# drapado/PINGS

Measured on AMD Instinct MI355X. Metric: raster fwd+bwd Mpix/s @1M Gaussians 1080p, higher is better.
Workload: dtype f32; 1 GPU; surfel rasteriser fwd+bwd, 1000000 Gaussians, 1920x1080, one view per GPU; gaussians=1000000, width=1920, height=1080

## Files before the change

include/pings_hip.h:

```cpp
#ifndef PINGS_HIP_H_
#define PINGS_HIP_H_

#include <stddef.h>
#include <stdint.h>

#if defined(__cplusplus)
#define PINGS_EXTERN_C extern "C"
#else
#define PINGS_EXTERN_C
#endif
#define PINGS_API PINGS_EXTERN_C __attribute__((visibility("default")))

#define PINGS_OK 0
#define PINGS_ERR_ARG 1
#define PINGS_ERR_HIP 2
#define PINGS_ERR_CAPACITY 3


#define PINGS_ABI_VERSION 11
PINGS_API int pings_abi_version(void);
PINGS_API const char* pings_last_error(void);

PINGS_API int pings_prof_enable(int on);
PINGS_API int pings_prof_only(const char* stage);
// ... 79 lines not shown
                                    void* bwd_blob, float* dL_dmeans3D, float* dL_dmeans2D,
                                    float* dL_dcolors, float* dL_dopacities, float* dL_dscales,
                                    float* dL_drotations, float* dL_dtau, int footprint_class,
                                    void* stream);

PINGS_API int pings_raster_debug_lists(const void* binning_blob, int64_t num_instances,
                                       int image_height, int image_width, uint32_t* point_list,
                                       uint32_t* ranges_xy, void* stream);
PINGS_API int pings_raster_debug_image(const void* image_blob, int image_height, int image_width,
                                       float* final_T, uint32_t* n_contrib, void* stream);
PINGS_API int pings_raster_debug_occlusion(const void* geom_blob, int P, int image_height, int image_width,
                                           uint32_t* occ_bucket, uint16_t* occ_bsat, int32_t* occ_nb,
                                           void* stream);
PINGS_API int pings_raster_rank_bucket(const int32_t* ranks, int64_t n, int occ_nb, uint32_t nvalid,
                                       uint32_t* buckets);
PINGS_API int pings_raster_debug_interior(const float* records, const float* tile_origins, int64_t n, float cxp,
                                          float cyp, float fx, float fy, uint8_t* flags);


PINGS_API size_t pings_raster2d_geom_bytes(int P, int image_height, int image_width);
PINGS_API size_t pings_raster2d_binning_bytes(int64_t num_instances, int image_height, int image_width);
PINGS_API size_t pings_raster2d_image_bytes(int image_height, int image_width);

PINGS_API int pings_raster2d_preprocess(const pings_raster_settings* s, int P, const float* means3D,
                                        const float* colors, const float* opacities, const float* scales,
                                        const float* rotations, void* geom_blob, int32_t* radii,
                                        const int32_t* live_rows_dev, int dyn_rows, const int32_t* const* aux_dev,
                                        int aux_words, int32_t* aux_host, int64_t* num_instances, void* stream);

PINGS_API int pings_raster2d_render(const pings_raster_settings* s, int P, int64_t num_instances, void* geom_blob,
// ... 814 lines not shown
```

pings_amd/_abi.py:

```python
from __future__ import annotations

import ctypes as C

ABI_VERSION = 11

RASTER_SURFEL, RASTER_3DGS, RASTER_2DGS = 0, 1, 2
HEAD_COLOR, HEAD_SEMANTIC = 0, 1
REG_SINGULAR, REG_ILL_CONDITIONED, REG_NONFINITE = 1, 2, 4
REG_F_NORMALS, REG_F_DIV_GRAD, REG_F_WEIGHTED = 1, 2, 4
REG_COLOR_PHOTO, REG_COLOR_CONSIST = 1, 2
MC_ALLOW_DEGENERATE, MC_ASCENT = 1, 2
ADAMW_MAX_JOBS, ADAMW_CHUNK = 48, 4096
EVAL_VIEW_RECORD, EVAL_PAIR_RECORD = 9, 12
EVAL_EXTENT = 1
MESH_SAMPLE_UNIT_BITS, MESH_SAMPLE_SUM_BITS = 32, 62
MESH_SAMPLE_INDEX, MESH_SAMPLE_NONFINITE, MESH_SAMPLE_AREA_CAP = 16, 32, 64
LOOP_MAX_R, LOOP_MAX_S, LOOP_MAX_D = 32, 128, 16
LOOP_MAX_Q, LOOP_MAX_C = 16, 65536
LIDAR_MAX_CAMS, LIDAR_MAX_LIDARS = 8, 8
CAMFRONT_MAX_MAPS, CAMFRONT_TILE_W, CAMFRONT_TILE_H = 32, 128, 32
CAMFRONT_RGB_U8, CAMFRONT_RGB_F32, CAMFRONT_NORMAL, CAMFRONT_DEPTH, CAMFRONT_SKY = 0, 1, 2, 3, 4
CAMFRONT_FIT_RECORD, CAMFRONT_MIN_FIT = 5, 100
CAMFRONT_FULL = 2
TSDF_BLOCK = 8
# ... 186 lines not shown
                                      C.POINTER(i32), vp]),
    "pings_raster_preprocess_dyn": (i32, [C.POINTER(RasterSettings), i32, vp, vp, vp, vp, vp, vp, vp, vp, i32,
                                          C.POINTER(vp), i32, C.POINTER(i32), C.POINTER(i64), C.POINTER(i32), vp]),
    "pings_raster_render": (i32, [C.POINTER(RasterSettings), i32, i64, vp, vp, vp, vp, vp, vp, vp, vp, i32, vp]),
    "pings_raster_tile_sort_bytes": (sz, [i64, C.POINTER(i32)]),
    "pings_raster_tile_sort": (i32, [vp, i64, i32, i32, vp, vp, vp, i32, vp]),
    "pings_raster_scan_bytes": (sz, [i64]),
    "pings_raster_scan_u32": (i32, [vp, i64, i32, i32, vp, vp, sz, vp]),
    "pings_raster_backward_bytes": (sz, [i32, i64]),
    "pings_raster_backward": (i32, [C.POINTER(RasterSettings), i32, i64, vp, vp, vp, vp, vp, vp, vp, vp, vp, vp, vp, vp,
                                    vp, vp, vp, vp, vp, vp, vp, vp, vp, vp, vp, vp, i32, vp]),
    "pings_raster_debug_lists": (i32, [vp, i64, i32, i32, vp, vp, vp]),
    "pings_raster_debug_image": (i32, [vp, i32, i32, vp, vp, vp]),
    "pings_raster_debug_occlusion": (i32, [vp, i32, i32, i32, vp, vp, C.POINTER(C.c_int32), vp]),
    "pings_raster_rank_bucket": (i32, [vp, i64, i32, C.c_uint32, vp]),
    "pings_raster_debug_interior": (i32, [vp, vp, i64, f32, f32, f32, f32, vp]),
    "pings_raster2d_geom_bytes": (sz, [i32, i32, i32]),
    "pings_raster2d_binning_bytes": (sz, [i64, i32, i32]),
    "pings_raster2d_image_bytes": (sz, [i32, i32]),
    "pings_raster2d_preprocess": (i32, [C.POINTER(RasterSettings), i32, vp, vp, vp, vp, vp, vp, vp, vp, i32,
                                        C.POINTER(vp), i32, C.POINTER(i32), C.POINTER(i64), vp]),
    "pings_raster2d_render": (i32, [C.POINTER(RasterSettings), i32, i64, vp, vp, vp, vp, vp, vp]),
    "pings_raster2d_backward_bytes": (sz, [i32, i64]),
    "pings_raster2d_backward": (i32, [C.POINTER(RasterSettings), i32, i64, vp, vp, vp, vp, vp, vp, vp, vp, vp, vp, vp,
                                      vp, vp, vp, vp]),
    "pings_raster2d_debug_lists": (i32, [vp, i64, i32, i32, vp, vp, vp]),
    "pings_raster2d_debug_image": (i32, [vp, i32, i32, vp, vp, vp, vp]),
    "pings_knn_compact_entries": (sz, [i64]),
    "pings_knn_compact_build": (i32, [vp, i64, vp, sz, vp]),
    "pings_knn_blocks_entries": (sz, [i64]),
# ... 192 lines not shown
```

pings_amd/csrc/raster_common.hpp:

```cpp
#pragma once
#include <cmath>
#include <cstdlib>
#include <type_traits>

#include "common.hpp"

namespace pings {
namespace raster {

constexpr int TILE = 16;
constexpr int BLOCK = TILE * TILE;
constexpr float NEAR_Z = 0.2f;
constexpr float LOWPASS = 0.3f;
constexpr float ALPHA_MAX = 0.99f;
constexpr float ALPHA_MIN = 1.0f / 255.0f;
constexpr float T_EPS = 1e-4f;
constexpr float DEPTH_ALPHA_EPS = 1e-10f;
constexpr float DEN_EPS = 1e-6f;
constexpr uint32_t CULLED_KEY = 0xFFFFFFFFu;
constexpr int DS_NB = 1 << 20;
constexpr uint32_t DS_LIMIT = 4096u;
constexpr int DS_SHARDS = 64;
constexpr int DS_KMIN = 2 * DS_SHARDS, DS_SHIFT = DS_KMIN + 1, DS_FLAG = DS_KMIN + 2, DS_HEAD = DS_KMIN + 8;
constexpr int STAT_SHARDS = 256;
// ... 5 lines not shown
constexpr uint16_t OCC_ALL = 0xFFFFu;

constexpr int MODE_SURFEL = 0;
constexpr int MODE_3DGS = 1;
constexpr int RECT_TIGHT = 0, RECT_3SIGMA = 1, RECT_ELLIPSE = 2;

constexpr int GRAD_ROW = 16;
constexpr int CH = 64;
enum GradSlot {
  G_MX = 0, G_MY = 1, G_CONX = 2, G_CONY = 3, G_CONZ = 4, G_OPAC = 5,
  G_R = 6, G_G = 7, G_B = 8, G_NX = 9, G_NY = 10, G_NZ = 11, G_Q = 12, G_PZ = 13,
  G_ZLO = 14, G_ZHI = 15
};

struct FrameSummary {
  uint32_t overflow, pad0;
  unsigned long long stats[3];
  int32_t aux[8];
  uint32_t seq;
  uint32_t pad;
};

struct GeomState {
  float4* rec;
  uint4* rect;
  uint32_t *depth_key, *depth_key_sorted, *gidx, *gidx_sorted;
  uint32_t* rank_of;
  uint32_t *tiles_sorted, *offsets_sorted;
  uint32_t* occ_bucket;
  uint16_t* occ_bsat;
  unsigned long long* occ_mask;
  uint32_t* nvalid;
  uint32_t* occ_bmax;
  uint32_t* ds_head;
  uint32_t *ds_cnt, *ds_fill, *ds_off;
  char* zero_begin; size_t zero_bytes;
  size_t ds_words;
  uint32_t* ds_idx;
  unsigned long long* stats;
  FrameSummary* summary;
  int occ_nb, occ_words;
  char* temp;
  size_t temp_bytes;
  size_t total;
};

struct BinState {
  uint32_t *tile_key, *tile_key_sorted, *gval, *point_list;
// ... 86 lines not shown
  uint32_t blend_seg = 512u;
  bool seg_reuse = true;
  uint32_t bwd_long = 3072u;
  bool occlusion = true;
  bool library_sort = false;
  bool library_tile_sort = false;
  bool library_scan = false;
  float occ_amin = 0.15f;
  bool occ_walk_lanes = false;
  int rect_rule = RECT_TIGHT;
  bool mark_depth_only = false;
  unsigned rowsum_wgs = 2048u;
  unsigned grad_fill_wgs = 512u;
  bool chain_sum_lanes = false;
  bool blend_interior = true;
};
RasterKnobs read_knobs();

struct BlendPlan {
  enum Fwd { FWD_TILE, FWD_WAVE } fwd;
  bool want_qmask;
  bool bwd_scan;
  uint32_t seg;
  bool seg_on, seg_reuse;
  uint32_t long_thr;
  bool interior_bwd;
};
BlendPlan blend_plan(const RasterKnobs& k, int footprint_class, int64_t I, int num_tiles);

struct BwdState {
// ... 11 lines not shown
                      uint32_t long_thr = 0, uint32_t long_max = 0);
int occlusion_buckets(int num_tiles);
BinState carve_binning(void* blob, int64_t I, int num_tiles, uint32_t seg);
ImageState carve_image(void* blob, int W, int H);
BwdState carve_bwd(void* blob, int P, int64_t I);

constexpr int TS_THREADS = 256, TS_BLOCK = 4096;
size_t tile_sort_table_bytes(int64_t n);
template <typename KeyT>
int tile_sort(const KeyT* keys_in, int64_t n, int bits, KeyT* keys_tmp, uint32_t* vals_tmp, KeyT* keys_out,
              uint32_t* vals_out, uint32_t* table, hipStream_t st);
size_t tile_sort_library_bytes(int64_t n);
template <typename KeyT>
int tile_sort_library(const KeyT* keys_in, int64_t n, int bits, KeyT* keys_out, uint32_t* vals_out, void* temp,
                      size_t temp_bytes, hipStream_t st);

int launch_blend_fwd(int mode, const KParams& kp, const BlendPlan& plan, int P, int64_t I, const GeomState& gs,
                     const BinState& bs, const ImageState& im, float* out_color, float* out_normal, float* out_depth,
                     float* out_alpha, void* per_gaussian, hipStream_t st);

__device__ inline int lane_value(int v, int src) { return __builtin_amdgcn_readlane(v, src); }
__device__ inline uint32_t lane_value(uint32_t v, int src) { return (uint32_t)__builtin_amdgcn_readlane((int)v, src); }
__device__ inline float lane_value(float v, int src) {
  return __builtin_bit_cast(float, __builtin_amdgcn_readlane(__builtin_bit_cast(int, v), src));
}

__device__ inline int dealt_rank(int num_waves, int wave, int lane) {
  return lane < 16 ? lane * num_waves + wave : ((lane >> 4) * num_waves + wave) * 16 + (lane & 15);
}
__device__ inline int strided_rank(int P) {
// ... 13 lines not shown
  uint32_t J = 0u;
  if ((eq >> RB_LW) != 0u) {
    J = rank_bucket_log2(eq >> RB_LW) + 2u;
    if (J > (unb >> (RB_LS + 1))) J = unb >> (RB_LS + 1);
  }
  const uint32_t front_ranks = J ? 1u << (RB_LW + RB_LS + J - 1u) : 0u, front_buckets = J << RB_LS;
  if (ur < front_ranks) {
    const uint32_t q = ur >> RB_LW;
    if ((q >> RB_LS) == 0u) return q;
    const uint32_t k = rank_bucket_log2(q) - RB_LS;
    return (k << RB_LS) + (q >> k);
  }
  const uint32_t b = front_buckets + (uint32_t)(((unsigned long long)(ur - front_ranks) * (unb - front_buckets)) /
                                                (unsigned long long)(nvalid - front_ranks));
  return b < unb ? b : unb - 1u;
}

typedef float f2 __attribute__((ext_vector_type(2)));
__device__ inline f2 f2s(float x) { return f2{x, x}; }
__device__ inline f2 fma2(f2 a, f2 b, f2 c) { return __builtin_elementwise_fma(a, b, c); }
__device__ inline f2 mul_rounded(f2 a, f2 b) {
#pragma clang fp contract(off)
  return a * b;
}
__device__ inline f2 sel2(bool c0, bool c1, f2 a, f2 b) { return f2{c0 ? a.x : b.x, c1 ? a.y : b.y}; }

typedef unsigned long long lmask;
struct cmask {
  unsigned long long bits;
};
// ... 390 lines not shown
```

pings_amd/csrc/raster_fwd.hip:

```cpp
#include <hipcub/hipcub.hpp>

#include <algorithm>
#include <chrono>
#include <type_traits>

#include "raster_common.hpp"

namespace pings {
namespace raster {

__device__ inline void to_camera(const float* __restrict__ V, float x, float y, float z, float& px,
                                 float& py, float& pz) {
  px = ((V[0] * x + V[4] * y) + V[8] * z) + V[12];
  py = ((V[1] * x + V[5] * y) + V[9] * z) + V[13];
  pz = ((V[2] * x + V[6] * y) + V[10] * z) + V[14];
}

__global__ __launch_bounds__(256) void mark_visible_kernel(const float* __restrict__ pos, int N,
                                                            const float* __restrict__ V,
                                                            const float* __restrict__ Pm,
                                                            uint8_t* __restrict__ present, int depth_only) {
  const int i = blockIdx.x * blockDim.x + threadIdx.x;
  if (i >= N) return;
  float px, py, pz;
// ... 254 lines not shown
  if (r >= 0 && (uint32_t)r < nvalid) {
    me.g = gidx_sorted[r];
    const uint4 rc = rect[me.g];
    me.n = rc.w;
    me.xmin = (int)(rc.y & 0xFFFF);
    me.ymin = (int)(rc.y >> 16);
    me.wdt = max((int)(rc.z & 0xFFFF) - me.xmin, 1);
    me.hgt = max((int)(rc.z >> 16) - me.ymin, 1);
  }
  return me;
}

constexpr int SMALL_ITEMS = 16;
constexpr uint32_t SMALL_KEPT = 16u;

__device__ inline unsigned long long kept_bits(const unsigned long long* __restrict__ m, int s, int w) {
  const int i = s >> 6, sh = s & 63;
  const unsigned long long lo = m[i], hi = m[i + 1];
  const unsigned long long v = sh ? (lo >> sh) | (hi << (64 - sh)) : lo;
  return v & (~0ull >> (64 - w));
}

struct RowItems {
  int s0, gx, wdt, cpr;
  float inv_cpr;
  __device__ RowItems(int xmin, int ymin, int wdt_, int gx_)
      : s0(ymin * gx_ + xmin), gx(gx_), wdt(wdt_), cpr((wdt_ + 63) >> 6), inv_cpr(1.0f / (float)((wdt_ + 63) >> 6)) {}
  __device__ void at(uint32_t k, int& s, int& w) const {
    int y = (int)k, c = 0;
    if (cpr > 1) {
      y = (int)((float)k * inv_cpr);
      c = (int)k - y * cpr;
      if (c < 0) { --y; c += cpr; }
      if (c >= cpr) { ++y; c -= cpr; }
    }
    s = s0 + y * gx + 64 * c;
// ... 444 lines not shown
                     n_long, long_thr, long_max);
  PINGS_LAUNCH_CHECK();
  return PINGS_OK;
}

template <typename KeyT>
__global__ __launch_bounds__(256) void tile_ranges_kernel(int64_t I, const KeyT* __restrict__ key,
                                                           uint2* __restrict__ ranges) {
  const int64_t i = (int64_t)blockIdx.x * blockDim.x + threadIdx.x;
  if (i >= I) return;
  const uint32_t t = (uint32_t)key[i];
  if (i == 0 || key[i - 1] != t) ranges[t].x = (uint32_t)i;
  if (i == I - 1 || key[i + 1] != t) ranges[t].y = (uint32_t)(i + 1);
}

struct AuxPtrs {
  const int32_t* p[8];
};
__global__ __launch_bounds__(64) void frame_summary_kernel(const uint32_t* __restrict__ overflow,
                                                           const unsigned long long* __restrict__ shards, AuxPtrs aux,
                                                           int aux_words, FrameSummary* __restrict__ out, uint32_t seq) {
  __shared__ unsigned long long part[3][64];
  const int lane = threadIdx.x;
  unsigned long long a0 = 0, a1 = 0, a2 = 0;
  for (int i = lane; i < STAT_SHARDS; i += 64) {
    a0 += shards[STAT_PAIRS + i]; a1 += shards[STAT_VISIBLE + i]; a2 += shards[STAT_KEPT + i];
  }
  part[0][lane] = a0; part[1][lane] = a1; part[2][lane] = a2;
  __syncthreads();
  if (lane < 3) {
    unsigned long long t = 0;
    for (int i = 0; i < 64; ++i) t += part[lane][i];
    out->stats[lane] = t;
  }
  if (lane == 4) out->overflow = overflow ? *overflow : 0u;
  if (lane >= 8 && lane < 16) out->aux[lane - 8] = (lane - 8 < aux_words && aux.p[lane - 8]) ? *aux.p[lane - 8] : 0;
  __threadfence_system();
  __syncthreads();
  if (lane == 0) __hip_atomic_store(&out->seq, seq, __ATOMIC_RELEASE, __HIP_MEMORY_SCOPE_SYSTEM);
}

static int make_params(const pings_raster_settings* s, int P, const RasterKnobs& knobs, KParams& kp) {
  if (int e = fill_camera(s, P, kp)) return e;
  kp.occ_amin = knobs.occ_amin;
  kp.rect_rule = knobs.rect_rule;
  kp.live = nullptr;
  kp.dyn_rows = 0;
  return PINGS_OK;
}

static int tile_bits(int num_tiles) {
  int b = 1;
  while ((1 << b) < num_tiles) ++b;
  return b;
}

}
}

using namespace pings::raster;

PINGS_API int pings_raster_mark_visible(const float* positions, int N,
                                        const pings_raster_settings* s, uint8_t* present,
// ... 4 lines not shown
  const int depth_only = read_knobs().mark_depth_only;
  hipLaunchKernelGGL(mark_visible_kernel, dim3(pings::ceil_div(N, 256)), dim3(256), 0,
                     pings::as_stream(stream), positions, N, s->viewmatrix, s->projmatrix_raw,
                     present, depth_only);
  PINGS_LAUNCH_CHECK();
  return PINGS_OK;
}

PINGS_API int pings_raster_rank_bucket(const int32_t* ranks, int64_t n, int occ_nb, uint32_t nvalid,
                                       uint32_t* buckets) {
  PINGS_ARG_CHECK(n >= 0 && occ_nb > 0 && (n == 0 || (ranks && buckets)), "null pointer / non-positive bucket count");
  for (int64_t i = 0; i < n; ++i) buckets[i] = rank_bucket(ranks[i], occ_nb, nvalid);
  return PINGS_OK;
}

PINGS_API int pings_raster_debug_interior(const float* records, const float* tile_origins, int64_t n, float cxp,
                                          float cyp, float fx, float fy, uint8_t* flags) {
  PINGS_ARG_CHECK(n >= 0 && (n == 0 || (records && tile_origins && flags)), "null pointer / negative count");
  PINGS_ARG_CHECK(fx > 0.f && fy > 0.f, "non-positive focal length");
  for (int64_t i = 0; i < n; ++i) {
    const float* r = records + 16 * i;
    const float X0 = tile_origins[2 * i], Y0 = tile_origins[2 * i + 1];
    flags[i] = blend_interior(r[0], r[1], r[2], r[3], r[4], r[5], r[6], r[7], r[11], r[12], r[13], r[14], X0, Y0,
                              tile_rays(X0, Y0, cxp, cyp, fx, fy)) ? 1 : 0;
  }
  return PINGS_OK;
}

PINGS_API int pings_raster_preprocess(const pings_raster_settings* s, int P, const float* means3D,
                                      const float* colors, const float* opacities,
// ... 4 lines not shown
                                     nullptr, 0, nullptr, num_instances, footprint_class, stream);
}

PINGS_API int pings_raster_preprocess_dyn(const pings_raster_settings* s, int P, const float* means3D,
                                          const float* colors, const float* opacities, const float* scales,
                                          const float* rotations, void* geom_blob, int32_t* radii,
                                          const int32_t* live_rows_dev, int dyn_rows,
                                          const int32_t* const* aux_dev, int aux_words, int32_t* aux_host,
                                          int64_t* num_instances, int32_t* footprint_class, void* stream) {
  const RasterKnobs knobs = read_knobs();
  KParams kp;
  if (int e = make_params(s, P, knobs, kp)) return e;
  PINGS_ARG_CHECK(num_instances != nullptr && footprint_class != nullptr, "null output");
  *num_instances = 0;
  *footprint_class = 1;
  PINGS_ARG_CHECK(aux_words >= 0 && aux_words <= 8 && (aux_words == 0 || (aux_dev && aux_host)), "0..8 aux words");
  PINGS_ARG_CHECK(!live_rows_dev || (dyn_rows >= 0 && dyn_rows <= P), "dyn_rows must lie in 0..P");
  PINGS_ARG_CHECK(P > 0 || aux_words == 0, "aux words need a non-empty frame");
  if (P == 0) return PINGS_OK;
  kp.live = live_rows_dev;
  kp.dyn_rows = live_rows_dev ? dyn_rows : 0;
  PINGS_ARG_CHECK(P > 0 && means3D && colors && opacities && scales && rotations && geom_blob && radii,
                  "null pointer");
  hipStream_t st = pings::as_stream(stream);
  const int num_tiles = kp.gx * kp.gy;
  GeomState gs = carve_geom(geom_blob, P, num_tiles);
  const dim3 grid(pings::ceil_div(P, 256)), block(256);
  const bool occlusion = knobs.occlusion;
  bool library_sort = knobs.library_sort;
  PINGS_HIP_CHECK(hipMemsetAsync(gs.zero_begin, 0, gs.zero_bytes, st));
// ... 58 lines not shown
      if (attempt > 0)
        PINGS_HIP_CHECK(hipMemsetAsync(gs.stats + STAT_KEPT, 0, STAT_RETRY_WORDS * sizeof(unsigned long long), st));
      hipLaunchKernelGGL(occl_scan_kernel, dim3(gs.occ_words), dim3(512), 0, st, num_tiles, gs.occ_nb, gs.occ_bucket,
                         gs.occ_bsat, gs.occ_mask, gs.occ_bmax);
      PINGS_LAUNCH_CHECK();
    }
    {
      pings::prof::Scope ps("tile_count_scan", st);
      hipLaunchKernelGGL(count_kept_kernel, grid, block, 0, st, P, kp.gx, gs.occ_nb, gs.occ_words, gs.gidx_sorted,
                         gs.rect, gs.occ_mask, gs.nvalid, gs.occ_bmax, gs.tiles_sorted, gs.stats);
      PINGS_LAUNCH_CHECK();
    }
    const uint32_t seq = ++frame_seq ? frame_seq : ++frame_seq;
    hipLaunchKernelGGL(frame_summary_kernel, dim3(1), dim3(64), 0, st,
                       library_sort ? (const uint32_t*)nullptr : gs.ds_head + DS_FLAG, gs.stats, aux, aux_words,
                       host_sum_dev, seq);
    PINGS_LAUNCH_CHECK();
    {
      pings::prof::Scope ps("tile_count_scan", st);
      if (int e = raster_scan_u32(gs.tiles_sorted, P, true, gs.offsets_sorted, gs.temp, gs.temp_bytes, knobs.library_scan, st))
        return e;
    }
    {
      const auto t_start = std::chrono::steady_clock::now();
      unsigned spins = 0;
      while (__atomic_load_n(&host_sum->seq, __ATOMIC_ACQUIRE) != seq) {
        if ((++spins & 0x3FFu) == 0) {
          const hipError_t q = hipStreamQuery(st);
          if (q == hipErrorNotReady) (void)hipGetLastError();
          else if (q != hipSuccess) PINGS_HIP_CHECK(q);
          if (std::chrono::steady_clock::now() - t_start > std::chrono::seconds(20)) {
            PINGS_HIP_CHECK(hipStreamSynchronize(st));
            PINGS_ARG_CHECK(__atomic_load_n(&host_sum->seq, __ATOMIC_ACQUIRE) == seq, "frame summary never arrived");
          }
        }
        __builtin_ia32_pause();
      }
    }
    if (host_sum->overflow == 0) break;
    library_sort = true;
  }
  const unsigned long long stats[3] = {host_sum->stats[0], host_sum->stats[1], host_sum->stats[2]};
  for (int i = 0; i < aux_words; ++i) aux_host[i] = host_sum->aux[i];
  PINGS_ARG_CHECK(stats[2] < 0x7FFFFFFFull, "more than 2^31 - 1 (Gaussian, tile) instances in this frame");
  *num_instances = (int64_t)stats[2];
  *footprint_class = (stats[1] > 0 && stats[0] > 16ull * stats[1]) ? 2 : 1;
  return PINGS_OK;
}

PINGS_API int pings_raster_render(const pings_raster_settings* s, int P, int64_t I,
                                  void* geom_blob, void* binning_blob, void* image_blob,
                                  float* out_color, float* out_normal,
                                  float* out_depth, float* out_alpha, void* per_gaussian,
                                  int footprint_class, void* stream) {
  const RasterKnobs knobs = read_knobs();
  KParams kp;
  if (int e = make_params(s, P, knobs, kp)) return e;
  PINGS_ARG_CHECK(out_color && out_depth && out_alpha && image_blob && binning_blob, "null pointer");
  PINGS_ARG_CHECK(s->mode == PINGS_RASTER_3DGS || out_normal, "surfel mode needs out_normal");
  PINGS_ARG_CHECK(I >= 0 && I < (int64_t)0x7FFFFFFF, "instance count out of range");
  PINGS_ARG_CHECK(P == 0 || (geom_blob && per_gaussian), "null pointer");
  hipStream_t st = pings::as_stream(stream);
  const int num_tiles = kp.gx * kp.gy;
  GeomState gs = carve_geom(geom_blob, P, num_tiles);
  BinState bs = carve_binning(binning_blob, I, num_tiles, knobs.blend_seg);
  ImageState im = carve_image(image_blob, kp.W, kp.H);

  {
    const char* z0 = reinterpret_cast<const char*>(bs.ranges);
    const char* z1 = I > 0 ? (s->mode == PINGS_RASTER_3DGS ? reinterpret_cast<const char*>(bs.inst_cnt + I)
                                                             : reinterpret_cast<const char*>(bs.inst_qmask + I + 1))
                           : reinterpret_cast<const char*>(bs.ranges + num_tiles);
    PINGS_HIP_CHECK(hipMemsetAsync(bs.ranges, 0, pings::align_up((size_t)(z1 - z0)), st));
  }
  if (I > 0) {
    auto bin = [&](auto* key, auto* key_sorted) -> int {
      using KeyT = std::remove_pointer_t<decltype(key)>;
      {
        pings::prof::Scope ps("duplicate", st);
        hipLaunchKernelGGL(duplicate_kernel<KeyT>, dim3(pings::ceil_div(P, 256)), dim3(256), 0, st, P,
                           kp.gx, gs.occ_nb, gs.occ_words, gs.gidx_sorted, gs.offsets_sorted, gs.tiles_sorted,
                           gs.rect, gs.occ_mask, gs.nvalid, key, bs.gval, reinterpret_cast<uint32_t*>(per_gaussian));
        PINGS_LAUNCH_CHECK();
      }
      const int bits = tile_bits(num_tiles);
      const KeyT* sorted = key_sorted;
      {
        pings::prof::Scope ps("tile_sort", st);
        if (knobs.library_tile_sort || bits > 16) {
          if (int e = tile_sort_library<KeyT>(key, I, bits, key_sorted, bs.point_list, bs.temp, bs.temp_bytes, st)) return e;
// ... 4 lines not shown
            return e;
        }
      }
      {
        pings::prof::Scope ps("tile_ranges", st);
        hipLaunchKernelGGL(tile_ranges_kernel<KeyT>, dim3((unsigned)pings::ceil_div<int64_t>(I, 256)), dim3(256), 0,
                           st, I, sorted, bs.ranges);
        PINGS_LAUNCH_CHECK();
      }
      return PINGS_OK;
    };
    const int e = num_tiles <= 65536 ? bin(reinterpret_cast<uint16_t*>(bs.tile_key), reinterpret_cast<uint16_t*>(bs.tile_key_sorted))
                                     : bin(bs.tile_key, bs.tile_key_sorted);
    if (e) return e;
  }
  {
    pings::prof::Scope ps_o("tile_order", st);
    hipLaunchKernelGGL(tile_order_kernel<true>, dim3(1), dim3(1024), 0, st, (const uint32_t*)nullptr, bs.ranges, num_tiles,
                       bs.tile_order, (uint32_t*)nullptr, 0u, 0u);
    PINGS_LAUNCH_CHECK();
  }
  return launch_blend_fwd(s->mode, kp, blend_plan(knobs, footprint_class, I, num_tiles), P, I, gs, bs, im, out_color,
                          out_normal, out_depth, out_alpha, per_gaussian, st);
}
```

pings_amd/csrc/raster_layout.hip:

```cpp
#include <hipcub/hipcub.hpp>

#include <algorithm>
#include <cmath>
#include <cstdlib>
#include <cstring>

#include "raster_common.hpp"

namespace pings {
namespace raster {

static size_t sort_temp_bytes(int64_t n) {
  size_t a = 0, b = 0;
  (void)hipcub::DeviceRadixSort::SortPairs(nullptr, a, (uint32_t*)nullptr, (uint32_t*)nullptr,
                                     (uint32_t*)nullptr, (uint32_t*)nullptr, (int)n, 0, 32);
  (void)hipcub::DeviceScan::InclusiveSum(nullptr, b, (uint32_t*)nullptr, (uint32_t*)nullptr,
                                         (int)std::max<int64_t>(n, DS_NB + n / 256 + 2));
  size_t c = 0;
  (void)hipcub::DeviceRadixSort::SortPairs(nullptr, c, (uint16_t*)nullptr, (uint16_t*)nullptr,
                                           (uint32_t*)nullptr, (uint32_t*)nullptr, (int)n, 0, 16);
  if (c > a) a = c;
  a = std::max(a, std::max(tile_sort_library_bytes(n), tile_sort_table_bytes(n)));
  a = std::max(a, raster_scan_bytes(std::max<int64_t>(n, DS_NB + n / 256 + 2)));
  return align_up(a > b ? a : b) + 256;
// ... 11 lines not shown
  const size_t n = (size_t)(P > 0 ? P : 1);
  const size_t nt = (size_t)(num_tiles > 0 ? num_tiles : 1);
  g.rec = c.take<float4>(4 * n);
  g.rect = c.take<uint4>(n);
  g.depth_key = c.take<uint32_t>(n);
  g.depth_key_sorted = c.take<uint32_t>(n);
  g.gidx = c.take<uint32_t>(n);
  g.gidx_sorted = c.take<uint32_t>(n);
  g.rank_of = c.take<uint32_t>(n);
  g.tiles_sorted = c.take<uint32_t>(n);
  g.offsets_sorted = c.take<uint32_t>(n);
  g.occ_nb = occlusion_buckets((int)nt);
  g.occ_bucket = c.take<uint32_t>(nt * (size_t)g.occ_nb);
  g.stats = c.take<unsigned long long>(STAT_WORDS);
  g.occ_bmax = g.stats ? reinterpret_cast<uint32_t*>(g.stats + STAT_BMAX) : nullptr;
  const size_t nblk = (n + 255) / 256;
  g.ds_words = DS_HEAD + (size_t)DS_NB + nblk;
  g.ds_head = c.take<uint32_t>(g.ds_words);
  g.ds_cnt = g.ds_head ? g.ds_head + DS_HEAD : nullptr;
  g.zero_begin = reinterpret_cast<char*>(g.occ_bucket);
  g.zero_bytes = g.ds_head ? align_up((size_t)(reinterpret_cast<char*>(g.ds_head + g.ds_words) - g.zero_begin)) : 0;
  g.occ_bsat = c.take<uint16_t>(nt);
  g.occ_words = (int)((nt + 63) / 64);
  g.occ_mask = c.take<unsigned long long>((size_t)g.occ_nb * (size_t)g.occ_words + 1);
  g.nvalid = c.take<uint32_t>(1);
  g.ds_off = c.take<uint32_t>((size_t)DS_NB + nblk + 1);
  g.ds_idx = c.take<uint32_t>(n);
  g.summary = c.take<FrameSummary>(1);
  g.temp_bytes = sort_temp_bytes((int64_t)n);
  g.temp = c.take<char>(g.temp_bytes);
// ... 73 lines not shown
    const long v = atol(e);
    k.bwd_long = v <= 0 ? 0xFFFFFFF0u : (uint32_t)((v + 15) / 16 * 16);
  }
  if (const char* e = getenv("PINGS_RASTER_OCCLUSION")) k.occlusion = atoi(e) != 0;
  if (const char* e = getenv("PINGS_DEPTH_SORT")) k.library_sort = e[0] == 'l';
  if (const char* e = getenv("PINGS_TILE_SORT")) k.library_tile_sort = e[0] == 'l';
  if (const char* e = getenv("PINGS_RASTER_SCAN")) k.library_scan = e[0] == 'l';
  if (const char* e = getenv("PINGS_OCC_AMIN")) k.occ_amin = fminf(fmaxf((float)atof(e), 1.0f / 255.0f), 0.99f);
  if (const char* e = getenv("PINGS_OCC_WALK")) k.occ_walk_lanes = e[0] == 'l';
  if (const char* e = getenv("PINGS_RASTER_RECT")) k.rect_rule = e[0] == '3' ? RECT_3SIGMA : e[0] == 'e' ? RECT_ELLIPSE : RECT_TIGHT;
  if (const char* e = getenv("PINGS_MARK_VISIBLE")) k.mark_depth_only = e[0] == 'd';
  if (const char* e = getenv("PINGS_ROWSUM_WGS")) k.rowsum_wgs = (unsigned)std::min(std::max(atoi(e), 1), 65535);
  if (const char* e = getenv("PINGS_GRAD_FILL")) k.grad_fill_wgs = e[0] == 'l' ? 0u : (unsigned)std::min(std::max(atoi(e), 1), 65535);
  if (const char* e = getenv("PINGS_CHAIN_SUM")) k.chain_sum_lanes = e[0] == 'l';
  if (const char* e = getenv("PINGS_BLEND_INTERIOR")) k.blend_interior = atoi(e) != 0;
  return k;
}

BlendPlan blend_plan(const RasterKnobs& k, int footprint_class, int64_t I, int num_tiles) {
  BlendPlan p;
  p.bwd_scan = k.blend_bwd == RasterKnobs::BWD_AUTO ? footprint_class != 2 : k.blend_bwd == RasterKnobs::BWD_SCAN;
  p.want_qmask = p.bwd_scan;
  const bool tile_wave = k.blend_ppl == 4 || (k.blend_ppl == 0 && footprint_class == 2 && !p.want_qmask);
  p.fwd = tile_wave ? BlendPlan::FWD_TILE : BlendPlan::FWD_WAVE;
  p.seg = k.blend_seg;
  p.seg_on = p.seg > 0 && I > (int64_t)num_tiles * (p.seg / 4) && I > 2 * (int64_t)p.seg;
  p.seg_reuse = p.seg <= 65535u && k.seg_reuse;
  p.long_thr = k.bwd_long;
  p.interior_bwd = k.blend_interior;
  return p;
// ... 77 lines not shown
```

Baseline: 2838 Mpix/s.

## Add gather-based tile binning path as alternative to key sort for dense frames

Adds a binning path that skips the (tile, depth) key radix sort. Each tile instead gathers its instances from a depth-ordered front of Gaussians, using the occlusion masks and per-row prefix bases. The frame summary kernel now also finds the front length, and the host picks gather when the frame is in footprint class 2 and a cost estimate favours it. The price is extra kernels, two passes (count, then fill) over the front for every tile, and a dependence on occlusion-mask state; whether it beats the sort depends on front size.

```diff
diff --git a/include/pings_hip.h b/include/pings_hip.h
--- a/include/pings_hip.h
+++ b/include/pings_hip.h
@@ -117,6 +117,7 @@
                                            void* stream);
 PINGS_API int pings_raster_rank_bucket(const int32_t* ranks, int64_t n, int occ_nb, uint32_t nvalid,
                                        uint32_t* buckets);
+PINGS_API int pings_raster_debug_bin_plan(int32_t* plan, uint32_t* front);
 PINGS_API int pings_raster_debug_interior(const float* records, const float* tile_origins, int64_t n, float cxp,
                                           float cyp, float fx, float fy, uint8_t* flags);
 
diff --git a/pings_amd/_abi.py b/pings_amd/_abi.py
--- a/pings_amd/_abi.py
+++ b/pings_amd/_abi.py
@@ -224,6 +224,7 @@
     "pings_raster_debug_image": (i32, [vp, i32, i32, vp, vp, vp]),
     "pings_raster_debug_occlusion": (i32, [vp, i32, i32, i32, vp, vp, C.POINTER(C.c_int32), vp]),
     "pings_raster_rank_bucket": (i32, [vp, i64, i32, C.c_uint32, vp]),
+    "pings_raster_debug_bin_plan": (i32, [C.POINTER(i32), C.POINTER(C.c_uint32)]),
     "pings_raster_debug_interior": (i32, [vp, vp, i64, f32, f32, f32, f32, vp]),
     "pings_raster2d_geom_bytes": (sz, [i32, i32, i32]),
     "pings_raster2d_binning_bytes": (sz, [i64, i32, i32]),
diff --git a/pings_amd/csrc/raster_common.hpp b/pings_amd/csrc/raster_common.hpp
--- a/pings_amd/csrc/raster_common.hpp
+++ b/pings_amd/csrc/raster_common.hpp
@@ -43,7 +43,7 @@
 };
 
 struct FrameSummary {
-  uint32_t overflow, pad0;
+  uint32_t overflow, front;
   unsigned long long stats[3];
   int32_t aux[8];
   uint32_t seq;
@@ -61,6 +61,7 @@
   unsigned long long* occ_mask;
   uint32_t* nvalid;
   uint32_t* occ_bmax;
+  uint32_t* occ_front;
   uint32_t* ds_head;
   uint32_t *ds_cnt, *ds_fill, *ds_off;
   char* zero_begin; size_t zero_bytes;
@@ -177,6 +178,8 @@
   unsigned grad_fill_wgs = 512u;
   bool chain_sum_lanes = false;
   bool blend_interior = true;
+  enum Bin { BIN_AUTO, BIN_SORT, BIN_GATHER };
+  Bin bin = BIN_AUTO;
 };
 RasterKnobs read_knobs();
 
@@ -218,6 +221,17 @@
 template <typename KeyT>
 int tile_sort_library(const KeyT* keys_in, int64_t n, int bits, KeyT* keys_out, uint32_t* vals_out, void* temp,
                       size_t temp_bytes, hipStream_t st);
+
+constexpr uint32_t FRONT_MAX = 8192u;
+constexpr int GATHER_CHUNK = 2048;
+constexpr uint64_t GATHER_COST = 25u;
+constexpr uint32_t FRONT_UNKNOWN = 0xFFFFFFFFu;
+inline bool gather_fits(uint32_t front, int gx, int gy, int nb, int64_t I) {
+  return front >= 1u && front <= FRONT_MAX && gx <= 256 && gy <= 256 && nb <= 256 && (int64_t)front * gy <= 2 * I &&
+         2 * (int64_t)front <= I;
+}
+int launch_tile_gather(const KParams& kp, int P, int64_t I, uint32_t front, const GeomState& gs, const BinState& bs,
+                       void* per_gaussian, hipStream_t st);
 
 int launch_blend_fwd(int mode, const KParams& kp, const BlendPlan& plan, int P, int64_t I, const GeomState& gs,
                      const BinState& bs, const ImageState& im, float* out_color, float* out_normal, float* out_depth,
@@ -261,6 +275,13 @@
   const uint32_t b = front_buckets + (uint32_t)(((unsigned long long)(ur - front_ranks) * (unb - front_buckets)) /
                                                 (unsigned long long)(nvalid - front_ranks));
   return b < unb ? b : unb - 1u;
+}
+
+__device__ inline unsigned long long kept_bits(const unsigned long long* __restrict__ m, int s, int w) {
+  const int i = s >> 6, sh = s & 63;
+  const unsigned long long lo = m[i], hi = m[i + 1];
+  const unsigned long long v = sh ? (lo >> sh) | (hi << (64 - sh)) : lo;
+  return v & (~0ull >> (64 - w));
 }
 
 typedef float f2 __attribute__((ext_vector_type(2)));
diff --git a/pings_amd/csrc/raster_fwd.hip b/pings_amd/csrc/raster_fwd.hip
--- a/pings_amd/csrc/raster_fwd.hip
+++ b/pings_amd/csrc/raster_fwd.hip
@@ -292,12 +292,6 @@
 constexpr int SMALL_ITEMS = 16;
 constexpr uint32_t SMALL_KEPT = 16u;
 
-__device__ inline unsigned long long kept_bits(const unsigned long long* __restrict__ m, int s, int w) {
-  const int i = s >> 6, sh = s & 63;
-  const unsigned long long lo = m[i], hi = m[i + 1];
-  const unsigned long long v = sh ? (lo >> sh) | (hi << (64 - sh)) : lo;
-  return v & (~0ull >> (64 - w));
-}
 
 struct RowItems {
   int s0, gx, wdt, cpr;
@@ -772,13 +766,20 @@
   if (i == I - 1 || key[i + 1] != t) ranges[t].y = (uint32_t)(i + 1);
 }
 
+constexpr int FRONT_SCAN_STEPS = 16;
+enum { FRONT_NEVER = 0, FRONT_CLASS2 = 1, FRONT_ALWAYS = 2 };
 struct AuxPtrs {
   const int32_t* p[8];
 };
 __global__ __launch_bounds__(64) void frame_summary_kernel(const uint32_t* __restrict__ overflow,
                                                            const unsigned long long* __restrict__ shards, AuxPtrs aux,
-                                                           int aux_words, FrameSummary* __restrict__ out, uint32_t seq) {
+                                                           int aux_words, FrameSummary* __restrict__ out, uint32_t seq,
+                                                           int nb, const uint32_t* __restrict__ nvalid,
+                                                           const uint32_t* __restrict__ bmax,
+                                                           const uint32_t* __restrict__ tiles_sorted,
+                                                           uint32_t* __restrict__ front, int front_mode) {
   __shared__ unsigned long long part[3][64];
+  __shared__ unsigned long long tot[3];
   const int lane = threadIdx.x;
   unsigned long long a0 = 0, a1 = 0, a2 = 0;
   for (int i = lane; i < STAT_SHARDS; i += 64) {
@@ -790,8 +791,45 @@
     unsigned long long t = 0;
     for (int i = 0; i < 64; ++i) t += part[lane][i];
     out->stats[lane] = t;
-  }
+    tot[lane] = t;
+  }
+  __syncthreads();
   if (lane == 4) out->overflow = overflow ? *overflow : 0u;
+  const bool want_front = front_mode == FRONT_ALWAYS || (front_mode == FRONT_CLASS2 && tot[1] > 0ull && tot[0] > 16ull * tot[1]);
+  if (!want_front) {
+    if (lane == 5) { out->front = FRONT_UNKNOWN; *front = FRONT_UNKNOWN; }
+  } else {
+    const uint32_t nv = *nvalid, bm = *bmax;
+    uint32_t lo = 0u, hi = nv;
+    if (bm + 1u >= (uint32_t)nb) lo = nv;
+    while (lo < hi) {
+      const uint32_t step = (hi - lo + 63u) / 64u;
+      const uint32_t pos = lo + (uint32_t)lane * step;
+      const bool le = pos < hi && rank_bucket((int)pos, nb, nv) <= bm;
+      const int nle = __popcll(__ballot(le));
+      if (nle == 0) { hi = lo; break; }
+      const uint32_t last_le = lo + (uint32_t)(nle - 1) * step;
+      lo = last_le + 1u;
+      hi = min(hi, last_le + step);
+    }
+    uint32_t fr = lo;
+    for (int step = 0; step < FRONT_SCAN_STEPS && fr > 0u; ++step) {
+      const uint32_t base = fr > 256u ? fr - 256u : 0u;
+      uint32_t last = 0u;
+#pragma unroll
+      for (uint32_t u = 0u; u < 4u; ++u) {
+        const uint32_t r = base + 64u * u + (uint32_t)lane;
+        if (r < fr && tiles_sorted[r] != 0u) last = r + 1u;
+      }
+#pragma unroll
+      for (int o = 32; o > 0; o >>= 1) last = max(last, (uint32_t)__shfl_xor((int)last, o, 64));
+      if (last != 0u) { fr = last; break; }
+      if (base == 0u) { fr = 0u; break; }
+      if (step + 1 < FRONT_SCAN_STEPS) fr = base;
+      else fr = lo;
+    }
+    if (lane == 5) { out->front = fr; *front = fr; }
+  }
   if (lane >= 8 && lane < 16) out->aux[lane - 8] = (lane - 8 < aux_words && aux.p[lane - 8]) ? *aux.p[lane - 8] : 0;
   __threadfence_system();
   __syncthreads();
@@ -805,6 +843,26 @@
   kp.live = nullptr;
   kp.dyn_rows = 0;
   return PINGS_OK;
+}
+
+struct FrontRecord {
+  const void* geom = nullptr;
+  int P = 0, num_tiles = 0;
+  int64_t I = 0;
+  uint32_t front = 0;
+};
+static thread_local FrontRecord t_front;
+static thread_local int t_bin_plan = 0;
+
+static bool plan_gather(const RasterKnobs& knobs, const void* geom_blob, int P, int64_t I, int footprint_class,
+                        const KParams& kp) {
+  const FrontRecord& fr = t_front;
+  const int num_tiles = kp.gx * kp.gy;
+  if (knobs.bin == RasterKnobs::BIN_SORT || I <= 0) return false;
+  if (fr.geom != geom_blob || fr.P != P || fr.I != I || fr.num_tiles != num_tiles) return false;
+  if (!gather_fits(fr.front, kp.gx, kp.gy, occlusion_buckets(num_tiles), I)) return false;
+  if (knobs.bin == RasterKnobs::BIN_GATHER) return true;
+  return footprint_class == 2 && (uint64_t)fr.front * (uint64_t)num_tiles <= GATHER_COST * (uint64_t)I;
 }
 
 static int tile_bits(int num_tiles) {
@@ -839,6 +897,13 @@
   return PINGS_OK;
 }
 
+PINGS_API int pings_raster_debug_bin_plan(int32_t* plan, uint32_t* front) {
+  PINGS_ARG_CHECK(plan && front, "null pointer");
+  *plan = t_bin_plan;
+  *front = t_front.front;
+  return PINGS_OK;
+}
+
 PINGS_API int pings_raster_debug_interior(const float* records, const float* tile_origins, int64_t n, float cxp,
                                           float cyp, float fx, float fy, uint8_t* flags) {
   PINGS_ARG_CHECK(n >= 0 && (n == 0 || (records && tile_origins && flags)), "null pointer / negative count");
@@ -873,6 +938,7 @@
   PINGS_ARG_CHECK(num_instances != nullptr && footprint_class != nullptr, "null output");
   *num_instances = 0;
   *footprint_class = 1;
+  t_front = FrontRecord{};
   PINGS_ARG_CHECK(aux_words >= 0 && aux_words <= 8 && (aux_words == 0 || (aux_dev && aux_host)), "0..8 aux words");
   PINGS_ARG_CHECK(!live_rows_dev || (dyn_rows >= 0 && dyn_rows <= P), "dyn_rows must lie in 0..P");
   PINGS_ARG_CHECK(P > 0 || aux_words == 0, "aux words need a non-empty frame");
@@ -961,7 +1027,8 @@
     const uint32_t seq = ++frame_seq ? frame_seq : ++frame_seq;
     hipLaunchKernelGGL(frame_summary_kernel, dim3(1), dim3(64), 0, st,
                        library_sort ? (const uint32_t*)nullptr : gs.ds_head + DS_FLAG, gs.stats, aux, aux_words,
-                       host_sum_dev, seq);
+                       host_sum_dev, seq, gs.occ_nb, gs.nvalid, gs.occ_bmax, gs.tiles_sorted, gs.occ_front,
+                       knobs.bin == RasterKnobs::BIN_SORT ? FRONT_NEVER : knobs.bin == RasterKnobs::BIN_GATHER ? FRONT_ALWAYS : FRONT_CLASS2);
     PINGS_LAUNCH_CHECK();
     {
       pings::prof::Scope ps("tile_count_scan", st);
@@ -991,6 +1058,11 @@
   for (int i = 0; i < aux_words; ++i) aux_host[i] = host_sum->aux[i];
   PINGS_ARG_CHECK(stats[2] < 0x7FFFFFFFull, "more than 2^31 - 1 (Gaussian, tile) instances in this frame");
   *num_instances = (int64_t)stats[2];
+  t_front.geom = geom_blob;
+  t_front.P = P;
+  t_front.num_tiles = num_tiles;
+  t_front.I = (int64_t)stats[2];
+  t_front.front = host_sum->front;
   *footprint_class = (stats[1] > 0 && stats[0] > 16ull * stats[1]) ? 2 : 1;
   return PINGS_OK;
 }
@@ -1020,7 +1092,11 @@
                            : reinterpret_cast<const char*>(bs.ranges + num_tiles);
     PINGS_HIP_CHECK(hipMemsetAsync(bs.ranges, 0, pings::align_up((size_t)(z1 - z0)), st));
   }
-  if (I > 0) {
+  const bool gather = plan_gather(knobs, geom_blob, P, I, footprint_class, kp);
+  t_bin_plan = gather ? 1 : 0;
+  if (gather) {
+    if (int e = launch_tile_gather(kp, P, I, t_front.front, gs, bs, per_gaussian, st)) return e;
+  } else if (I > 0) {
     auto bin = [&](auto* key, auto* key_sorted) -> int {
       using KeyT = std::remove_pointer_t<decltype(key)>;
       {
@@ -1055,7 +1131,7 @@
                                      : bin(bs.tile_key, bs.tile_key_sorted);
     if (e) return e;
   }
-  {
+  if (!gather) {
     pings::prof::Scope ps_o("tile_order", st);
     hipLaunchKernelGGL(tile_order_kernel<true>, dim3(1), dim3(1024), 0, st, (const uint32_t*)nullptr, bs.ranges, num_tiles,
                        bs.tile_order, (uint32_t*)nullptr, 0u, 0u);
diff --git a/pings_amd/csrc/raster_gather.hip b/pings_amd/csrc/raster_gather.hip
--- /dev/null
+++ b/pings_amd/csrc/raster_gather.hip
@@ -0,0 +1,203 @@
+#include <algorithm>
+
+#include "raster_common.hpp"
+
+namespace pings {
+namespace raster {
+
+constexpr uint32_t FRONT_EMPTY = 0xFFFFFFFFu;
+constexpr int GATHER_WAVES = 16;
+constexpr int GATHER_THREADS = GATHER_WAVES * 64;
+
+__global__ __launch_bounds__(256) void front_rows_kernel(int P, int gx, int nb, int words, uint32_t front_cap, int64_t I,
+                                                         int rank_blocks, const uint32_t* __restrict__ gidx_sorted,
+                                                         const uint32_t* __restrict__ offsets_sorted,
+                                                         const uint32_t* __restrict__ tiles_sorted,
+                                                         const uint4* __restrict__ rect,
+                                                         const unsigned long long* __restrict__ mask,
+                                                         const uint32_t* __restrict__ nvalid,
+                                                         const uint32_t* __restrict__ front_dev,
+                                                         uint2* __restrict__ entries, uint32_t* __restrict__ rowbase,
+                                                         uint32_t* __restrict__ gval,
+                                                         uint32_t* __restrict__ per_gaussian) {
+  if ((int)blockIdx.x >= rank_blocks) {
+    const size_t stride = (size_t)(gridDim.x - rank_blocks) * 256u;
+    for (size_t i = (size_t)((int)blockIdx.x - rank_blocks) * 256u + threadIdx.x; i < (size_t)P; i += stride)
+      per_gaussian[i] = 0u;
+    return;
+  }
+  const int lane = threadIdx.x & 63;
+  const uint32_t r = blockIdx.x * 4u + (threadIdx.x >> 6);
+  if (r >= min(*front_dev, front_cap)) return;
+  const uint32_t kept = tiles_sorted[r];
+  const uint32_t bk = rank_bucket((int)r, nb, *nvalid);
+  if (kept == 0u) {
+    if (lane == 0) entries[r] = make_uint2(FRONT_EMPTY, bk | (r << 8));
+    return;
+  }
+  const uint32_t g = gidx_sorted[r];
+  const uint4 rc = rect[g];
+  const int xmin = (int)(rc.y & 0xFFFF), ymin = (int)(rc.y >> 16);
+  const int wdt = max((int)(rc.z & 0xFFFF) - xmin, 1), hgt = max((int)(rc.z >> 16) - ymin, 1);
+  if (lane == 0)
+    entries[r] = make_uint2((uint32_t)xmin | ((uint32_t)ymin << 8) | ((uint32_t)(wdt - 1) << 16) | ((uint32_t)(hgt - 1) << 24),
+                            bk | (r << 8));
+  const unsigned long long* mrow = mask + (size_t)bk * words;
+  const uint32_t first = offsets_sorted[r] - kept;
+  uint32_t run = first;
+  for (int y0 = 0; y0 < hgt; y0 += 64) {
+    const int y = y0 + lane;
+    uint32_t c = 0u;
+    if (y < hgt) {
+      const int s = (ymin + y) * gx + xmin;
+      for (int x = 0; x < wdt; x += 64) c += (uint32_t)__popcll(kept_bits(mrow, s + x, min(64, wdt - x)));
+    }
+    const uint32_t incl = wave_inclusive_sum_dpp(c);
+    if (y < hgt) rowbase[(size_t)(ymin + y) * front_cap + r] = run + (incl - c);
+    run += lane_value(incl, 63);
+  }
+  for (uint32_t i = (uint32_t)lane; i < kept; i += 64u)
+    if ((int64_t)first + i < I) gval[first + i] = g;
+}
+
+template <bool COUNT>
+__global__ __launch_bounds__(GATHER_THREADS) void tile_gather_kernel(int gx, int num_tiles, int words, uint32_t front_cap,
+                                                                     int64_t I, const uint32_t* __restrict__ front_dev,
+                                                                     const uint2* __restrict__ entries,
+                                                                     const uint32_t* __restrict__ rowbase,
+                                                                     const uint16_t* __restrict__ bsat,
+                                                                     const unsigned long long* __restrict__ mask,
+                                                                     uint32_t* __restrict__ counts,
+                                                                     uint2* __restrict__ ranges,
+                                                                     uint32_t* __restrict__ point_list,
+                                                                     uint32_t* __restrict__ order) {
+  __shared__ uint2 sEnt[GATHER_CHUNK];
+  __shared__ uint32_t sWave[GATHER_WAVES];
+  __shared__ uint32_t sSat[GATHER_WAVES];
+  const int lane = threadIdx.x & 63, wave = threadIdx.x >> 6;
+  int group = (int)blockIdx.x;
+  if constexpr (!COUNT) {
+    if (group == 0) {
+      tile_order_body<false>(counts, nullptr, num_tiles, order, nullptr, 0u, 0u);
+      return;
+    }
+    --group;
+  }
+  const int tile0 = group * GATHER_WAVES, tile = tile0 + wave;
+  const bool live = tile < num_tiles;
+  const uint32_t F = min(*front_dev, front_cap);
+  const int ty = live ? tile / gx : 0, tx = live ? tile - ty * gx : 0;
+  const uint32_t sat = live ? (uint32_t)bsat[tile] : 0u;
+  const int tlast = min(tile0 + GATHER_WAVES, num_tiles) - 1;
+  const int ty0 = tile0 / gx, ty1 = tlast / gx;
+  const int tx0 = ty0 == ty1 ? tile0 - ty0 * gx : 0, tx1 = ty0 == ty1 ? tlast - ty0 * gx : gx - 1;
+  if (lane == 0) sSat[wave] = live ? min(sat, 255u) : 0u;
+  uint32_t begin = 0u;
+  if constexpr (!COUNT) {
+    uint32_t s = 0u;
+    for (int t = (int)threadIdx.x; t < tile0; t += GATHER_THREADS) s += counts[t];
+    s = wave_reduce_sum_u32_dpp(s);
+    if (lane == 63) sWave[wave] = s;
+    __syncthreads();
+    const int t = tile0 + lane;
+    uint32_t b = lane < GATHER_WAVES ? sWave[lane] : 0u;
+    if (lane < wave && t < num_tiles) b += counts[t];
+    begin = lane_value(wave_reduce_sum_u32_dpp(b), 63);
+  }
+  __syncthreads();
+  uint32_t wgsat = 0u;
+#pragma unroll
+  for (int w = 0; w < GATHER_WAVES; ++w) wgsat = max(wgsat, sSat[w]);
+  uint32_t running = 0u;
+  bool done = !live;
+  for (uint32_t c0 = 0u; c0 < F; c0 += (uint32_t)GATHER_CHUNK) {
+    const uint32_t n = min((uint32_t)GATHER_CHUNK, F - c0);
+    uint32_t ncomp = 0u;
+    for (uint32_t k0 = 0u; k0 < n; k0 += (uint32_t)GATHER_THREADS) {
+      const uint32_t k = k0 + threadIdx.x;
+      uint2 e = make_uint2(FRONT_EMPTY, 0u);
+      if (k < n) e = entries[c0 + k];
+      const int x0 = (int)(e.x & 255u), y0 = (int)((e.x >> 8) & 255u);
+      const int x1 = x0 + (int)((e.x >> 16) & 255u), y1 = y0 + (int)(e.x >> 24);
+      const bool keep = e.x != FRONT_EMPTY && (e.y & 255u) <= wgsat && y0 <= ty1 && y1 >= ty0 && x0 <= tx1 && x1 >= tx0;
+      const unsigned long long m = __ballot(keep);
+      __syncthreads();
+      if (lane == 0) sWave[wave] = (uint32_t)__popcll(m);
+      __syncthreads();
+      uint32_t at = ncomp, tot = 0u;
+#pragma unroll
+      for (int w = 0; w < GATHER_WAVES; ++w) {
+        const uint32_t c = sWave[w];
+        at += w < wave ? c : 0u;
+        tot += c;
+      }
+      if (keep) sEnt[at + (uint32_t)__popcll(m & ((1ull << lane) - 1ull))] = e;
+      ncomp += tot;
+    }
+    __syncthreads();
+    if (done) continue;
+    for (uint32_t k0 = 0u; k0 < ncomp; k0 += 64u) {
+      const uint32_t k = k0 + (uint32_t)lane;
+      const uint2 e = sEnt[min(k, ncomp - 1u)];
+      if ((lane_value(e.y, 0) & 255u) > sat) { done = true; break; }
+      const uint32_t dx = (uint32_t)tx - (e.x & 255u), dy = (uint32_t)ty - ((e.x >> 8) & 255u);
+      const bool hit = k < ncomp && (e.y & 255u) <= sat && dx <= ((e.x >> 16) & 255u) && dy <= (e.x >> 24);
+      const unsigned long long m = __ballot(hit);
+      if constexpr (!COUNT) {
+        if (hit) {
+          uint32_t slot = rowbase[(size_t)ty * front_cap + (e.y >> 8)];
+          if (dx != 0u) {
+            const unsigned long long* mrow = mask + (size_t)(e.y & 255u) * words;
+            const int s = tile - (int)dx;
+            for (int x = 0; x < (int)dx; x += 64) slot += (uint32_t)__popcll(kept_bits(mrow, s + x, min(64, (int)dx - x)));
+          }
+          const uint32_t pos = begin + running + (uint32_t)__popcll(m & ((1ull << lane) - 1ull));
+          if ((int64_t)pos < I) point_list[pos] = slot;
+        }
+      }
+      running += (uint32_t)__popcll(m);
+    }
+  }
+  if (live && lane == 0) {
+    if constexpr (COUNT) {
+      counts[tile] = running;
+    } else if (running != 0u) {
+      ranges[tile] = make_uint2(begin, begin + running);
+    }
+  }
+}
+
+int launch_tile_gather(const KParams& kp, int P, int64_t I, uint32_t front, const GeomState& gs, const BinState& bs,
+                       void* per_gaussian, hipStream_t st) {
+  const int num_tiles = kp.gx * kp.gy;
+  PINGS_ARG_CHECK(gather_fits(front, kp.gx, kp.gy, gs.occ_nb, I), "the gather tables do not fit this frame");
+  uint2* entries = reinterpret_cast<uint2*>(bs.slot_val);
+  uint32_t* rowbase = bs.tile_key;
+  uint32_t* counts = bs.tile_work;
+  {
+    pings::prof::Scope ps("front_rows", st);
+    const int rank_blocks = (int)pings::ceil_div<uint32_t>(front, 4u);
+    const int zero_blocks = std::min(std::max(pings::ceil_div(P, 2048), 1), 1024);
+    hipLaunchKernelGGL(front_rows_kernel, dim3(rank_blocks + zero_blocks), dim3(256), 0, st, P, kp.gx, gs.occ_nb,
+                       gs.occ_words, front, I, rank_blocks, gs.gidx_sorted, gs.offsets_sorted, gs.tiles_sorted, gs.rect,
+                       gs.occ_mask, gs.nvalid, gs.occ_front, entries, rowbase, bs.gval,
+                       reinterpret_cast<uint32_t*>(per_gaussian));
+    PINGS_LAUNCH_CHECK();
+  }
+  const int groups = pings::ceil_div(num_tiles, GATHER_WAVES);
+  {
+    pings::prof::Scope ps("tile_gather", st);
+    hipLaunchKernelGGL(tile_gather_kernel<true>, dim3(groups), dim3(GATHER_THREADS), 0, st, kp.gx, num_tiles,
+                       gs.occ_words, front, I, gs.occ_front, entries, rowbase, gs.occ_bsat, gs.occ_mask, counts, bs.ranges,
+                       bs.point_list, bs.tile_order);
+    PINGS_LAUNCH_CHECK();
+    hipLaunchKernelGGL(tile_gather_kernel<false>, dim3(groups + 1), dim3(GATHER_THREADS), 0, st, kp.gx, num_tiles,
+                       gs.occ_words, front, I, gs.occ_front, entries, rowbase, gs.occ_bsat, gs.occ_mask, counts, bs.ranges,
+                       bs.point_list, bs.tile_order);
+    PINGS_LAUNCH_CHECK();
+  }
+  return PINGS_OK;
+}
+
+}
+}
diff --git a/pings_amd/csrc/raster_layout.hip b/pings_amd/csrc/raster_layout.hip
--- a/pings_amd/csrc/raster_layout.hip
+++ b/pings_amd/csrc/raster_layout.hip
@@ -49,6 +49,7 @@
   g.occ_bucket = c.take<uint32_t>(nt * (size_t)g.occ_nb);
   g.stats = c.take<unsigned long long>(STAT_WORDS);
   g.occ_bmax = g.stats ? reinterpret_cast<uint32_t*>(g.stats + STAT_BMAX) : nullptr;
+  g.occ_front = g.occ_bmax ? g.occ_bmax + 1 : nullptr;
   const size_t nblk = (n + 255) / 256;
   g.ds_words = DS_HEAD + (size_t)DS_NB + nblk;
   g.ds_head = c.take<uint32_t>(g.ds_words);
@@ -152,6 +153,7 @@
   if (const char* e = getenv("PINGS_GRAD_FILL")) k.grad_fill_wgs = e[0] == 'l' ? 0u : (unsigned)std::min(std::max(atoi(e), 1), 65535);
   if (const char* e = getenv("PINGS_CHAIN_SUM")) k.chain_sum_lanes = e[0] == 'l';
   if (const char* e = getenv("PINGS_BLEND_INTERIOR")) k.blend_interior = atoi(e) != 0;
+  if (const char* e = getenv("PINGS_BIN")) k.bin = e[0] == 's' ? RasterKnobs::BIN_SORT : e[0] == 'g' ? RasterKnobs::BIN_GATHER : RasterKnobs::BIN_AUTO;
   return k;
 }
 
```

After: 2962 Mpix/s, median of 6. 4.4% higher.
